# trevor-m/cuda-pathtrace

Measured on AMD Instinct MI355X. Metric: Msamples/s, 9-sphere Cornell box 1024x1024x1024spp, higher is better.
Workload: dtype f32+f64

## Files before the change

### cuda-pathtrace_amd/csrc/pt_grid.h

```cpp
#pragma once
#include "pt_intersect.h"

#pragma clang fp contract(off)

namespace pt {

#ifndef PT_V13_LAST_SHORTCUT
#define PT_V13_LAST_SHORTCUT 1
#endif
#ifndef PT_GRID_MAX_CELLS
#define PT_GRID_MAX_CELLS 4096
#endif
#ifndef PT_GRID_CELLS_PER_SPHERE
#define PT_GRID_CELLS_PER_SPHERE 2.75f
#endif
#ifndef PT_GRID_EXACT_REG
#define PT_GRID_EXACT_REG 1
#endif
constexpr int kGridMaxCells = PT_GRID_MAX_CELLS;
#ifndef PT_GRID_TESTS_PER_TRIP
#define PT_GRID_TESTS_PER_TRIP 3
#endif
#ifndef PT_GRID_MAX_ITEMS
#define PT_GRID_MAX_ITEMS 8192
// ... 469 lines not shown
    h.far2 = far * far;
    h.n_big = n_big | ((ncells + n_ext) << 16);
    h.n_items = total;
    h.r_small = r_small;
    h.r_big = r_big;
    h.prim_base = (uint32_t)max_entries;
    h.n_emis = s_n_emis > (uint32_t)kGridMaxEmis ? 0xFFFFu : s_n_emis;
    *hdr = h;
  }
}

#ifdef PT_GRID_STATS
__device__ unsigned long long g_grid_stats[8];
__device__ unsigned long long g_grid_hist[4][64];
#define PT_HIST_DECL int hist_tests = 0, hist_steps = 0, hist_trips = 0, hist_rounds = 0
#define PT_HIST_LANE(var, n) do { var += (n); } while (0)
#define PT_HIST_END(in_walk) do { \
    if (in_walk) { atomicAdd(&g_grid_hist[0][hist_tests < 63 ? hist_tests : 63], 1ull); atomicAdd(&g_grid_hist[1][hist_steps < 63 ? hist_steps : 63], 1ull); } \
    if ((threadIdx.x & 63) == __builtin_ctzll(__builtin_amdgcn_ballot_w64(true))) { \
      atomicAdd(&g_grid_hist[2][hist_trips < 63 ? hist_trips : 63], 1ull); atomicAdd(&g_grid_hist[3][hist_rounds < 63 ? hist_rounds : 63], 1ull); } } while (0)
#define PT_STAT(i, v) do { const unsigned long long v_ = (unsigned long long)(v);  \
    if ((threadIdx.x & 63) == __builtin_ctzll(__builtin_amdgcn_ballot_w64(true))) atomicAdd(&g_grid_stats[i], v_); } while (0)
#else
#define PT_STAT(i, v) do { } while (0)
#define PT_HIST_DECL
#define PT_HIST_LANE(var, n) do { } while (0)
#define PT_HIST_END(in_walk) do { } while (0)
#endif
#ifdef PT_GRID_STATS_AMBIG
#define PT_STATW(i, v) do { } while (0)
#else
#define PT_STATW(i, v) PT_STAT(i, v)
#endif
struct Near2 {
  float T1, T2;
  int i1;
};

template <bool ONCE = false>
__device__ __forceinline__ bool near2_test(Near2& s, const float4 g, int i, F3 o, F3 d, float a4, float Tlim_hi) {
  const float INF = __builtin_inff();
  const F3 off = mk3(o.x - g.x, o.y - g.y, o.z - g.z);
  const float b = 2.0f * dot(d, off);
  const float c = dot(off, off) - g.w;
  const float bb = b * b;
  const float a4c = a4 * c;
  const float dacc = fmaf(-a4, c, bb);
  const bool cand = ((int)__float_as_uint(dacc) >= 0) & (ONCE || !((i == s.i1) & (s.T1 < INF)));
  const float sq = __builtin_amdgcn_sqrtf(dacc);
  const float e = fmaf(b, b, -bb);
  const float num = a4c + e;
  const float TA = copysign_neg_b3(sq, b) - b;
  const float TB = num * __builtin_amdgcn_rcpf(TA);
  const uint32_t ta = __float_as_uint(TA), tb = __float_as_uint(TB);
  const uint32_t tbits = ta < tb ? ta : tb;
  const float T = __uint_as_float(tbits);
  const bool sure = fabsf(a4c) > fmaf(bb, 1.1920929e-07f, 1e-30f);
  const bool ok = cand & sure & (tbits < __float_as_uint(Tlim_hi));
  const float Te = ok ? T : INF;
  s.i1 = Te < s.T1 ? i : s.i1;
  s.T2 = __builtin_amdgcn_fmed3f(s.T1, s.T2, Te);
  s.T1 = fminf(s.T1, Te);
  return cand & !sure;
}

__device__ __forceinline__ void near2_exact(Near2& s, const float4 g, int i, F3 o, F3 d, float a, float Tlim_hi) {
// ... 105 lines not shown
    const float tn = par[k] ? (inside ? -INF : INF) : fminf(l, h);
    const float tf = par[k] ? (inside ? INF : -INF) : fmaxf(l, h);
    t_in = fmaxf(t_in, tn);
    t_out = fminf(t_out, tf);
  }
  active = (t_in <= t_out + slack_t) & (t_in * two_a < Tlim_hi);
  const int stride[3] = {1, dims[0], dims[0] * dims[1]};
#pragma unroll
  for (int k = 0; k < 3; k++) {
    const float p = oo[k] + dd[k] * t_in;
    int ci = (int)floorf((p - gmin[k]) * G.h.inv_cs);
    ci = ci < 0 ? 0 : (ci >= dims[k] ? dims[k] - 1 : ci);
    const bool fwd = dd[k] > 0.0f;
    const float bnd = gmin[k] + (float)(ci + (fwd ? 1 : 0)) * G.h.cs;
    const float tm = par[k] ? INF : (bnd - oo[k]) * inv[k];
    const float td = par[k] ? INF : G.h.cs * fabsf(inv[k]);
    if (k == 0) { w.tmax0 = tm; w.tdel0 = td; }
    if (k == 1) { w.tmax1 = tm; w.tdel1 = td; }
    if (k == 2) { w.tmax2 = tm; w.tdel2 = td; }
    cidx += ci * stride[k];
    const int sk = fwd ? stride[k] : -stride[k];
    if (k == 0) w.cs0 = sk;
    if (k == 1) w.cs1 = sk;
    if (k == 2) w.cs2 = sk;
    left |= (uint32_t)(fwd ? dims[k] - 1 - ci : ci) << (10 * k);
  }
  cidx = active ? cidx : 0;
  }
  w.cidx = cidx;
  w.left = left;
  w.e0 = 0u, w.e1 = 0u;
  w.k0 = 0u, w.k1 = 0u;
  if constexpr (POOLED) {
    const uint2 e = G.cells[prim ? G.h.prim_base + (uint32_t)kPrimEntriesPerLane * threadIdx.x : (uint32_t)cidx];
    active = active & !settled;
    w.e0 = (active | prim) ? e.x : 0u;
    w.e1 = e.y;
    active = active & !prim;
  } else {
    w.k0 = G.cell_start[cidx], w.k1 = G.cell_start[cidx + 1];
    if (!active) w.k1 = w.k0;
  }
  w.n0 = 0, w.n1 = 0;
  w.have_next = false;
#ifdef PT_TIMING_ONLY_NO_WALK
  active = false;
  w.k1 = w.k0;
  w.e0 = 0u;
#endif
  w.walking = active;
  w.t_box = t_out + 2.0f * slack_t;
  w.forced = false;
  PT_STAT(0, 1);
  PT_STAT(5, __builtin_popcountll(__builtin_amdgcn_ballot_w64(active)));
}

template <bool PARK>
__device__ __forceinline__ void grid_trips(GridWalk& walk, const GridLds& G, F3 o, F3 d, bool in_walk, bool alive, int park) {
  const float two_a = 2.0f * walk.a, a4 = 4.0f * walk.a;
  const float Tlim_hi = 1000000.0f * two_a * 1.0000153f;
  const float slack_t = G.h.slack * __builtin_amdgcn_rsqf(walk.a);
  Near2 s = walk.s;
  float tmax0 = walk.tmax0, tmax1 = walk.tmax1, tmax2 = walk.tmax2;
  const float tdel0 = walk.tdel0, tdel1 = walk.tdel1, tdel2 = walk.tdel2;
  int cidx = walk.cidx;
  const int cs0 = walk.cs0, cs1 = walk.cs1, cs2 = walk.cs2;
  uint32_t left = walk.left, k0 = walk.k0, k1 = walk.k1, n0 = walk.n0, n1 = walk.n1;
// ... 123 lines not shown
  const float INF = __builtin_inff();
  return (dot(oc, oc) <= G.h.far2) & (a > 0.0f) & (a < 1e30f) & (fabsf(d.x) < INF) & (fabsf(d.y) < INF) & (fabsf(d.z) < INF);
}

__device__ __forceinline__ bool intersect_scene_v11(const SceneLds& sc, int n, F3 o, F3 d, float& t_hit, int& idx) {
  if (n <= 0) return false;
  const float a = dot(d, d);
  const GridLds& G = *sc.grid;
  if (G.valid) {
    const bool admitted = grid_admits(G, o, d, a);
    PT_STATW(7, __builtin_amdgcn_ballot_w64(!admitted) != 0 ? 1 : 0);
    if (admitted) return intersect_scene_grid(sc, G, n, o, d, a, t_hit, idx);
  }
  return intersect_scene_screened_large(sc, n, o, d, make_ray_const(d), t_hit, idx);
}

#ifndef PT_POOL_STEPS
#define PT_POOL_STEPS 2
#endif
#ifdef PT_DEBUG_PIXEL
#define PT_DBG_ME() (blockIdx.x == PT_DEBUG_BLOCK && threadIdx.x == PT_DEBUG_THREAD)
#define PT_DBG_MY_WAVE() (blockIdx.x == PT_DEBUG_BLOCK && (threadIdx.x >> 6) == (PT_DEBUG_THREAD >> 6))
#define PT_DBG_OWNED(owner) (PT_DBG_MY_WAVE() && (owner) == (PT_DEBUG_THREAD & 63))
#define PT_DBG(...) do { printf(__VA_ARGS__); } while (0)
#else
#define PT_DBG_ME() false
#define PT_DBG_MY_WAVE() false
#define PT_DBG_OWNED(owner) false
#define PT_DBG(...) do { } while (0)
#endif
#ifndef PT_POOL_SCAN_DPP
#define PT_POOL_SCAN_DPP 1
#endif
#ifndef PT_POOL_SWEEP_BELOW
#define PT_POOL_SWEEP_BELOW 24
#endif
static_assert(63 + 64 * 3 * PT_POOL_STEPS + 2 <= kPoolRing, "pool ring too small");
static_assert(PT_POOL_STEPS == 1 || PT_POOL_STEPS == 2, "the link queue has two slots");

struct PoolLds {
  uint32_t* ring;
  unsigned long long* key1;
  uint32_t* t2;
  uint32_t* olist;
  unsigned long long* smask;
};
constexpr unsigned long long kPoolEmpty = 0x7F800000FFFFFFFFull;

__device__ __forceinline__ PoolLds pool_of_wave(void* workgroup_base) {
  char* b = reinterpret_cast<char*>(workgroup_base) + (threadIdx.x >> 6) * kPoolWaveBytes;
  PoolLds p;
  p.key1 = reinterpret_cast<unsigned long long*>(b);
  p.ring = reinterpret_cast<uint32_t*>(b + 64 * 8);
  p.t2 = reinterpret_cast<uint32_t*>(b + 64 * 8 + kPoolRing * 4);
  p.olist = p.t2 + 64;
  p.smask = reinterpret_cast<unsigned long long*>(p.olist + 64);
  return p;
}

__device__ __forceinline__ float bperm_f(int byte_addr, float v) {
  return __int_as_float(__builtin_amdgcn_ds_bpermute(byte_addr, __float_as_int(v)));
}

__device__ __forceinline__ bool dda_step(float& tmax0, float& tmax1, float& tmax2, float tdel0, float tdel1, float tdel2, int& cidx,
                                         int cs0, int cs1, int cs2, float tstop) {
  const float t_exit = fminf(fminf(tmax0, tmax1), tmax2);
  const bool a0 = (tmax0 <= tmax1) & (tmax0 <= tmax2);
  const bool a1 = !a0 & (tmax1 <= tmax2);
  tmax0 = a0 ? tmax0 + tdel0 : tmax0;
  tmax1 = a1 ? tmax1 + tdel1 : tmax1;
  tmax2 = (a0 | a1) ? tmax2 : tmax2 + tdel2;
  cidx += a0 ? cs0 : (a1 ? cs1 : cs2);
  return t_exit <= tstop;
}

__device__ __forceinline__ void grid_trips_pooled(GridWalk& walk, const GridLds& G, const PoolLds& P, F3 o, F3 d) {
  constexpr int K = PT_POOL_STEPS;
  const float INF = __builtin_inff();
  const int lane = threadIdx.x & 63;
  const float a4 = 4.0f * walk.a;
  const float two_a = 2.0f * walk.a;
  const float slack_t = G.h.slack * __builtin_amdgcn_rsqf(walk.a);
  const float Tcap = 1000000.0f * two_a * 1.0000153f;
  const float inv_two_a = __builtin_amdgcn_rcpf(two_a);
  float tmax0 = walk.tmax0, tmax1 = walk.tmax1, tmax2 = walk.tmax2;
  const float tdel0 = walk.tdel0, tdel1 = walk.tdel1, tdel2 = walk.tdel2;
  int cidx = walk.cidx;
  const int cs0 = walk.cs0, cs1 = walk.cs1, cs2 = walk.cs2;
  const uint32_t last_cell = G.h.nx * G.h.ny * G.h.nz - 1u;
  const float t_box = walk.t_box;
  auto stop_at = [&](float best) { return fminf(fmaf(fminf(best * 1.0000077f, Tcap), inv_two_a, slack_t), t_box) * 1.0000019f; };
  bool walking = walk.walking;
  int rounds_left = (int)(G.h.nx + G.h.ny + G.h.nz) / K + 8 + (int)((G.h.n_big >> 16) - (last_cell + 1u));
  const uint64_t here = __builtin_amdgcn_ballot_w64(true);
  const uint32_t rank = __builtin_amdgcn_mbcnt_hi((uint32_t)(here >> 32), __builtin_amdgcn_mbcnt_lo((uint32_t)here, 0u));
  const uint32_t n_here = (uint32_t)__builtin_popcountll(here);
  __hip_atomic_store(P.key1 + lane, walk.s.T1 < INF ? (((unsigned long long)__float_as_uint(walk.s.T1) << 32) | (uint32_t)walk.s.i1) : kPoolEmpty,
                     __ATOMIC_RELAXED, __HIP_MEMORY_SCOPE_WORKGROUP);
  __hip_atomic_store(P.t2 + lane, __float_as_uint(walk.s.T2), __ATOMIC_RELAXED, __HIP_MEMORY_SCOPE_WORKGROUP);
  uint32_t links = 0u;
  uint32_t tail = 0u;
  float tstop = stop_at(walk.s.T1);
  PT_HIST_DECL;
  if (PT_DBG_ME()) PT_DBG("ENTRY walking %d tmax %g %g %g tdel %g %g %g cidx %d cs %d %d %d tstop %g t_box %g e0 %08x e1 %08x n_here %u T1 %g o %g %g %g d %g %g %g\n", (int)walking, tmax0, tmax1, tmax2, tdel0, tdel1, tdel2, cidx, cs0, cs1, cs2, tstop, t_box, walk.e0, walk.e1, n_here, walk.s.T1, o.x, o.y, o.z, d.x, d.y, d.z);
  auto push = [&](uint32_t e0k, uint32_t e1k, uint32_t tag, bool first) {
    const uint64_t m1 = __builtin_amdgcn_ballot_w64(e0k >= 0x40000000u);
    if (m1 != 0) {
      const uint64_t m2 = __builtin_amdgcn_ballot_w64(e0k >= 0x80000000u), m3 = __builtin_amdgcn_ballot_w64(e0k >= 0xC0000000u);
      uint32_t pos = __builtin_amdgcn_mbcnt_hi((uint32_t)(m1 >> 32), __builtin_amdgcn_mbcnt_lo((uint32_t)m1, tail));
      pos = __builtin_amdgcn_mbcnt_hi((uint32_t)(m2 >> 32), __builtin_amdgcn_mbcnt_lo((uint32_t)m2, pos));
      pos = __builtin_amdgcn_mbcnt_hi((uint32_t)(m3 >> 32), __builtin_amdgcn_mbcnt_lo((uint32_t)m3, pos));
      PT_HIST_LANE(hist_tests, (int)(e0k >> 30));
      if (e0k >= 0x40000000u) {
        uint32_t* slot = P.ring + pos;
        slot[2] = tag | (e1k >> 16);
        asm volatile("" ::: "memory");
        slot[1] = tag | (e1k & 0xFFFFu);
        asm volatile("" ::: "memory");
        slot[0] = tag | (e0k & 0xFFFFu);
      }
      tail += (uint32_t)(__builtin_popcountll(m1) + __builtin_popcountll(m2) + __builtin_popcountll(m3));
      if (first) links |= e0k & 0x1FFF0000u; else links |= (e0k >> 16) & 0x1FFFu;
    }
  };
  auto drain = [&](bool fin) {
  if (tail >= (fin ? 1u : n_here)) {
    uint32_t head = 0u;
    do {
      const uint32_t n = (tail - head) < n_here ? (tail - head) : n_here;
      const bool valid = rank < n;
      PT_STATW(1, 1);
      PT_STATW(2, n);
      PT_HIST_LANE(hist_trips, 1);
      const uint32_t e = P.ring[head + rank];
      head += n;
      const int owner = valid ? (int)(e >> 16) : lane;
      const int i = valid ? (int)(e & 0xFFFFu) : 0;
      const float4 g = G.geom[i];
      const int oa = owner << 2;
      const F3 ro = mk3(bperm_f(oa, o.x), bperm_f(oa, o.y), bperm_f(oa, o.z));
      const F3 rd = mk3(bperm_f(oa, d.x), bperm_f(oa, d.y), bperm_f(oa, d.z));
      const float ra4 = bperm_f(oa, a4);
      const float rTlim_hi = 1000000.0f * (0.5f * ra4) * 1.0000153f;
      const F3 off = mk3(ro.x - g.x, ro.y - g.y, ro.z - g.z);
      const float b = 2.0f * dot(rd, off);
      const float cc = dot(off, off) - g.w;
      const float bb = b * b;
      const float a4c = ra4 * cc;
      const float dacc = fmaf(-ra4, cc, bb);
      const bool cand = valid & ((int)__float_as_uint(dacc) >= 0);
      const float sq = __builtin_amdgcn_sqrtf(dacc);
      const float ee = fmaf(b, b, -bb);
      const float num = a4c + ee;
      const float TA = copysign_neg_b3(sq, b) - b;
      const float TB = num * __builtin_amdgcn_rcpf(TA);
      const uint32_t ta = __float_as_uint(TA), tb = __float_as_uint(TB);
      const uint32_t tbits = ta < tb ? ta : tb;
      float T = __uint_as_float(tbits);
      const bool sure = fabsf(a4c) > fmaf(bb, 1.1920929e-07f, 1e-30f);
      bool ok = cand & sure & (tbits < __float_as_uint(rTlim_hi));
      if (__builtin_expect(cand & !sure, 0)) {
        float t = 0.0f;
        const float ra = 0.25f * ra4;
        const bool h = intersect_sphere(ro, rd, ra, g, t);
        T = (2.0f * ra) * t;
        ok = h & (t > 0.0f) & (T < rTlim_hi);
      }
      if (ok) {
        const unsigned long long key = ((unsigned long long)__float_as_uint(T) << 32) | (uint32_t)i;
        const unsigned long long old = __hip_atomic_fetch_min(P.key1 + owner, key, __ATOMIC_RELAXED, __HIP_MEMORY_SCOPE_WORKGROUP);
        if (old != key) {
          const unsigned long long loser = old > key ? old : key;
          __hip_atomic_fetch_min(P.t2 + owner, (uint32_t)(loser >> 32), __ATOMIC_RELAXED, __HIP_MEMORY_SCOPE_WORKGROUP);
        }
      }
    } while ((tail - head) >= (fin ? 1u : n_here));
    const uint32_t rest = tail - head;
    if (rest != 0u) {
      const uint32_t v = P.ring[head + (rank < rest ? rank : 0u)];
      if (rank < rest) P.ring[rank] = v;
    }
    tail = rest;
    tstop = stop_at(__uint_as_float(__hip_atomic_load(reinterpret_cast<uint32_t*>(P.key1 + lane) + 1, __ATOMIC_RELAXED, __HIP_MEMORY_SCOPE_WORKGROUP)));
  }
  };

  uint32_t e0[K], e1[K];
  e0[0] = walk.e0, e1[0] = walk.e1;
#pragma unroll
  for (int k = 1; k < K; k++) e0[k] = 0u, e1[k] = 0u;
  const uint32_t self = (uint32_t)lane << 16;
  bool sweep = false;
  for (;;) {
#pragma unroll
    for (int k = 0; k < K; k++) push(e0[k], e1[k], self, k == 0);
    const bool fin = __builtin_amdgcn_ballot_w64(walking | (links != 0u)) == 0;
    drain(fin);
    if (fin) break;
    if (__builtin_expect(--rounds_left < 0, 0)) {
      walk.forced = walk.forced | walking | (links != 0u);
      walking = false;
      links = 0u;
    }
    if (n_here == 64u && __builtin_amdgcn_ballot_w64(links != 0u) == 0 &&
        __builtin_popcountll(__builtin_amdgcn_ballot_w64(walking)) <= PT_POOL_SWEEP_BELOW) {
      if (PT_DBG_ME()) PT_DBG("SWITCH walking %d walkers %d tmax %g %g %g cidx %d tstop %g rounds_left %d\n", (int)walking, (int)__builtin_popcountll(__builtin_amdgcn_ballot_w64(walking)), tmax0, tmax1, tmax2, cidx, tstop, rounds_left);
      sweep = true;
      break;
    }
    PT_STATW(3, 1);
    PT_STATW(4, __builtin_popcountll(__builtin_amdgcn_ballot_w64(walking | (links != 0u))));
    PT_HIST_LANE(hist_rounds, 1);
    uint32_t cur = 0u;
    if (__builtin_amdgcn_ballot_w64(links != 0u) != 0) {
      const uint32_t hi = links >> 16;
      cur = hi != 0u ? hi : links;
      links = hi != 0u ? (links & 0xFFFFu) : 0u;
    }
#pragma unroll
    for (int k = 0; k < K; k++) e0[k] = 0u, e1[k] = 0u;
    const bool chain = cur != 0u;
    bool go = chain;
    if (!chain & walking) {
      PT_HIST_LANE(hist_steps, 1);
      walking = dda_step(tmax0, tmax1, tmax2, tdel0, tdel1, tdel2, cidx, cs0, cs1, cs2, tstop);
      go = walking;
    }
    if (go) {
      const uint32_t at = (uint32_t)cidx < last_cell ? (uint32_t)cidx : last_cell;
      const uint2 e = G.cells[chain ? cur : at];
      e0[0] = e.x, e1[0] = e.y;
    }
    if (PT_DBG_ME()) PT_DBG("STEP0 walking %d chain %d cidx %d entry %08x %08x tmax %g %g %g\n", (int)walking, (int)chain, cidx, e0[0], e1[0], tmax0, tmax1, tmax2);
#pragma unroll
    for (int k = 1; k < K; k++) {
      if (!chain & walking) {
        PT_HIST_LANE(hist_steps, 1);
        walking = dda_step(tmax0, tmax1, tmax2, tdel0, tdel1, tdel2, cidx, cs0, cs1, cs2, tstop);
        if (walking) {
          const uint32_t at = (uint32_t)cidx < last_cell ? (uint32_t)cidx : last_cell;
          const uint2 e = G.cells[at];
          e0[k] = e.x, e1[k] = e.y;
        }
      }
    }
    if (PT_DBG_ME()) PT_DBG("STEP1 walking %d cidx %d entry %08x %08x tmax %g %g %g\n", (int)walking, cidx, e0[K - 1], e1[K - 1], tmax0, tmax1, tmax2);
  }
  if (sweep) {
    uint32_t sw_n = 0u, sw_total = 0u, sw_done = 0u;
    bool wide = false;
    if (walking) {
      auto crossings = [&](float tm, float td) {
        const int n = tm <= tstop ? (int)((tstop - tm) * __builtin_amdgcn_rcpf(td)) + 1 : 0;
        return (uint32_t)(n < 0 ? 0 : n);
      };
      const uint32_t n0 = crossings(tmax0, tdel0), n1 = crossings(tmax1, tdel1), n2 = crossings(tmax2, tdel2);
      wide = (n0 | n1 | n2) > 255u;
      sw_n = n0 | (n1 << 8) | (n2 << 16) | (cs0 < 0 ? 1u << 24 : 0u) | (cs1 < 0 ? 1u << 25 : 0u) | (cs2 < 0 ? 1u << 26 : 0u);
      sw_total = n0 + n1 + n2;
      if (PT_DBG_ME()) PT_DBG("COUNTS n %u %u %u\n", n0, n1, n2);
    }
    if (__builtin_expect(__builtin_amdgcn_ballot_w64(wide) != 0, 0)) {
      walk.forced = walk.forced | walking;
      sw_total = 0u;
    }
    uint32_t se0 = 0u, se1 = 0u, tag = self;
    for (;;) {
      se0 = 0u, se1 = 0u;
      if (__builtin_amdgcn_ballot_w64(links != 0u) != 0) {
        if (links != 0u) {
          const uint32_t hi = links >> 16, cur = hi != 0u ? hi : links;
          links = hi != 0u ? (links & 0xFFFFu) : 0u;
          const uint2 e = G.cells[cur];
          se0 = e.x, se1 = e.y;
        }
      } else {
        const uint32_t rem = sw_total - sw_done;
        uint32_t incl = rem;
#if PT_POOL_SCAN_DPP
// ... 31 lines not shown
        const bool serving = (uint32_t)lane < (served < 64u ? served : 64u);
        PT_STATW(3, 1);
        PT_STATW(4, served < 64u ? served : 64u);
        sw_done += take;
        const uint32_t info = P.olist[serving ? ray : 0u];
        const int oa = (int)(info & 0xFFu) << 2;
        const float m0 = bperm_f(oa, tmax0), m1 = bperm_f(oa, tmax1), m2 = bperm_f(oa, tmax2);
        const float d0 = bperm_f(oa, tdel0), d1 = bperm_f(oa, tdel1), d2 = bperm_f(oa, tdel2);
        const int base = __builtin_amdgcn_ds_bpermute(oa, cidx);
        const uint32_t nn = (uint32_t)__builtin_amdgcn_ds_bpermute(oa, (int)sw_n);
        if (serving) {
          const uint32_t li = (info >> 16) + ((uint32_t)lane - ((info >> 8) & 0xFFu));
          const uint32_t n0 = nn & 0xFFu, n1 = (nn >> 8) & 0xFFu;
          const bool k0 = li < n0, k1 = !k0 & (li < n0 + n1);
          const uint32_t i = li - (k0 ? 0u : (k1 ? n0 : n0 + n1));
          const float tc = (k0 ? m0 : (k1 ? m1 : m2)) + (float)i * (k0 ? d0 : (k1 ? d1 : d2));
          const int ax = k0 ? 0 : (k1 ? 1 : 2);
          auto taken = [&](float tmx, float td, int m) {
            const int j = tc >= tmx ? (int)((tc - tmx) * __builtin_amdgcn_rcpf(td) + 0.75f) : 0;
            const float tj = tmx + (float)j * td;
            return ((tj < tc) | ((tj == tc) & (m < ax))) ? j + 1 : j;
          };
          const int c0 = k0 ? (int)i + 1 : taken(m0, d0, 0), c1 = k1 ? (int)i + 1 : taken(m1, d1, 1),
                    c2 = (k0 | k1) ? taken(m2, d2, 2) : (int)i + 1;
          const int sx = (int)G.h.nx, sxy = (int)(G.h.nx * G.h.ny);
          const int idx = base + ((nn >> 24) & 1u ? -c0 : c0) + ((nn >> 25) & 1u ? -c1 : c1) * sx + ((nn >> 26) & 1u ? -c2 : c2) * sxy;
          const uint32_t at = (uint32_t)idx < last_cell ? (uint32_t)idx : last_cell;
          const uint2 e = G.cells[at];
          se0 = e.x, se1 = e.y;
          tag = (info & 0xFFu) << 16;
          if (PT_DBG_OWNED(info & 0xFFu)) PT_DBG("SERVE helper %d li %u axis %d i %u tc %g c %d %d %d base %d idx %d entry %08x %08x nn %08x\n", lane, li, k0 ? 0 : (k1 ? 1 : 2), i, tc, c0, c1, c2, base, idx, e.x, e.y, nn);
        }
      }
      push(se0, se1, tag, true);
      const bool fin = __builtin_amdgcn_ballot_w64((links != 0u) | (sw_done < sw_total)) == 0;
      drain(fin);
      if (fin) break;
    }
  }
  PT_HIST_END(true);
  const unsigned long long k = __hip_atomic_load(P.key1 + lane, __ATOMIC_RELAXED, __HIP_MEMORY_SCOPE_WORKGROUP);
  walk.s.T1 = __uint_as_float((uint32_t)(k >> 32));
  walk.s.i1 = walk.s.T1 < INF ? (int)(uint32_t)k : 0;
  walk.s.T2 = __uint_as_float(__hip_atomic_load(P.t2 + lane, __ATOMIC_RELAXED, __HIP_MEMORY_SCOPE_WORKGROUP));
  if (PT_DBG_ME()) PT_DBG("FINAL T1 %g i1 %d T2 %g forced %d swept %d\n", walk.s.T1, walk.s.i1, walk.s.T2, (int)walk.forced, (int)sweep);
}

__device__ __forceinline__ bool intersect_scene_grid_pooled(const SceneLds& sc, const GridLds& G, int n, F3 o, F3 d, float a,
                                                            float& t_hit, int& idx, bool walker = true, bool prim = false,
                                                            bool last = false) {
  GridWalk w;
  grid_begin<true>(w, G, o, d, a, prim & walker, last & walker);
  const float INF = __builtin_inff();
  w.s.T1 = walker ? w.s.T1 : INF;
  w.s.T2 = walker ? w.s.T2 : INF;
  w.walking = w.walking & walker;
  w.e0 = walker ? w.e0 : 0u;
  w.e1 = walker ? w.e1 : 0u;
  grid_trips_pooled(w, G, pool_of_wave(sc.pool), o, d);
  if (!walker) return false;
  return grid_end(w, sc, G, n, o, d, t_hit, idx);
}

__device__ __forceinline__ bool intersect_scene_v13(const SceneLds& sc, int n, F3 o, F3 d, float& t_hit, int& idx, bool live = true,
                                                    bool prim = false, bool last = false) {
  if (n <= 0) return false;
  const float a = dot(d, d);
  const GridLds& G = *sc.grid;
  if (G.valid) {
    const bool admitted = live && grid_admits(G, o, d, a);
    PT_STATW(7, __builtin_amdgcn_ballot_w64(live & !admitted) != 0 ? 1 : 0);
    const bool walk_here = __builtin_amdgcn_ballot_w64(admitted) != 0;
    if (admitted | (walk_here & !live)) {
// ... 10 lines not shown
```

### cuda-pathtrace_amd/csrc/pt_kernel.hip

```cpp
#include "pt_trace.h"

#pragma clang fp contract(off)

static constexpr int kNumVariants = 15;
static constexpr int kT = PT_BLOCK_THREADS, kTG = PT_GRID_BLOCK_THREADS, kTW = PT_GRID_WIDE_THREADS;
static constexpr int kW = PT_MIN_WAVES, kWG = PT_GRID_MIN_WAVES, kWD = PT_GRID12_MIN_WAVES, kWP = PT_POOL_MIN_WAVES;
static constexpr VariantInfo kVariants[kNumVariants] = {
     {true,  1, kT,  PT_LEAN_NEVER,  PT_LDS_PLAIN,  PT_GRID_NONE,   false, false, false, false, PT_CHUNK_NONE,     false, kW,   PT_LOOP_SAMPLES,   0,     0},
     {false, 1, kT,  PT_LEAN_NEVER,  PT_LDS_PLAIN,  PT_GRID_NONE,   false, false, false, false, PT_CHUNK_NONE,     false, kW,   PT_LOOP_SAMPLES,   1,     1},
     {false, 1, kT,  PT_LEAN_NEVER,  PT_LDS_PLAIN,  PT_GRID_NONE,   false, false, false, false, PT_CHUNK_NONE,     false, kW,   PT_LOOP_SAMPLES,   2,     2},
     {false, 1, kT,  PT_LEAN_NEVER,  PT_LDS_PACKED, PT_GRID_NONE,   false, false, false, false, PT_CHUNK_NONE,     false, kW,   PT_LOOP_SAMPLES,   3,     3},
     {false, 1, kT,  PT_LEAN_NEVER,  PT_LDS_PLAIN,  PT_GRID_NONE,   false, false, false, false, PT_CHUNK_NONE,     false, kW,   PT_LOOP_SAMPLES,   4,     4},
     {false, 1, kT,  PT_LEAN_NEVER,  PT_LDS_PLAIN,  PT_GRID_NONE,   false, false, false, false, PT_CHUNK_NONE,     false, kW,   PT_LOOP_SAMPLES,   5,     5},
     {true,  1, kT,  PT_LEAN_BIG,    PT_LDS_WALLS,  PT_GRID_NONE,   false, true,  true,  true,  PT_CHUNK_ONE_LANE, true,  kW,   PT_LOOP_SAMPLES,   6,     6},
     {false, 1, kT,  PT_LEAN_NEVER,  PT_LDS_PLAIN,  PT_GRID_NONE,   false, false, false, false, PT_CHUNK_NONE,     false, kW,   PT_LOOP_PAIRS,     6,     7},
     {true,  4, kT,  PT_LEAN_BIG,    PT_LDS_PLAIN,  PT_GRID_NONE,   false, true,  false, false, PT_CHUNK_SPLIT,    true,  0,    PT_LOOP_SAMPLES,   6,     8},
     {true,  2, kT,  PT_LEAN_NEVER,  PT_LDS_PLAIN,  PT_GRID_NONE,   false, true,  false, false, PT_CHUNK_SPLIT,    true,  0,    PT_LOOP_SAMPLES,   6,     9},
     {true,  1, kT,  PT_LEAN_BIG,    PT_LDS_PLAIN,  PT_GRID_NONE,   false, false, true,  false, PT_CHUNK_NONE,     false, kW,   PT_LOOP_REGEN,     6,     10},
     {false, 1, kTG, PT_LEAN_ALWAYS, PT_LDS_PLAIN,  PT_GRID_LANE,   false, false, false, false, PT_CHUNK_NONE,     false, kWG,  PT_LOOP_REGEN,     11,    11},
     {false, 1, kTG, PT_LEAN_ALWAYS, PT_LDS_PLAIN,  PT_GRID_LANE,   false, false, false, false, PT_CHUNK_NONE,     false, kWD,  PT_LOOP_DECOUPLED, 11,    12},
     {true,  1, kTG, PT_LEAN_ALWAYS, PT_LDS_PLAIN,  PT_GRID_POOLED, false, false, true,  false, PT_CHUNK_GRID,     true,  kWP,  PT_LOOP_REGEN,     13,    13},
     {true,  1, kTW, PT_LEAN_ALWAYS, PT_LDS_PLAIN,  PT_GRID_POOLED, true,  false, true,  false, PT_CHUNK_GRID,     false, kWP,  PT_LOOP_REGEN,     13,    13},
};
static constexpr VariantInfo kNoVariant = {false, 1, kT, PT_LEAN_NEVER, PT_LDS_PLAIN, PT_GRID_NONE, false, false, false, false, PT_CHUNK_NONE, false, kW, PT_LOOP_SAMPLES, 0, 0};
// ... 249 lines not shown
      sx /= (float)a.height;
      sy /= (float)a.width;
    }
    dir = lerp(lerp(B0, B1, sy), lerp(B2, B3, sy), 1.0f - sx);
  };

  auto dir_at = [&](float sx, float sy) {
    if (pow2_image) {
      sx *= inv_h;
      sy *= inv_w;
    } else {
      sx /= (float)a.height;
      sy /= (float)a.width;
    }
    return lerp(lerp(B0, B1, sy), lerp(B2, B3, sy), 1.0f - sx);
  };
  if constexpr (REF) {
#ifndef PT_NO_FOOTPRINT
    if (pass_spp >= PT_FOOTPRINT_MIN_SPP) {
      const uint32_t mine = active ? primary_candidates(sc, a.n_spheres, (float)row, (float)col, dir_at) : 0u;
      uint32_t wave_mask = 0u;
#pragma unroll
      for (int j = 0; j < 9; j++) wave_mask |= (__builtin_amdgcn_ballot_w64(((mine >> j) & 1u) != 0u) != 0ull) ? (1u << j) : 0u;
      sc.prim_mask = wave_mask;
    }
#endif
  }

  int i = active ? i_begin : i_end;
  bool prim_ok = false;
  if constexpr (POOLED && PT_PRIMLIST) {
    if (grid.valid && pass_spp >= PT_PRIMLIST_MIN_SPP && a.max_bounces >= 1) {
      int k = 0;
      const uint32_t slot = grid.h.prim_base + (uint32_t)kPrimEntriesPerLane * threadIdx.x;
      prim_ok = build_primary_list(grid, a.spheres, a.n_spheres, eye, (float)row, (float)col, active, dir_at, pool_of_wave(sc.pool).ring,
                                   const_cast<uint2*>(grid.cells), slot, k);
      if (prim_ok & (k == 0) & ((grid.h.n_big & 0xFFFFu) == 0u)) {
        for (; i < i_end; i++) {
          if constexpr (RNG == PT_RNG_XORWOW) {
            if (RESUME || a.spp != 1) {
              float jx, jy;
              rng.jitter(jx, jy);
            }
          }
          L.color = L.color + mk3(0.0f, 0.0f, 0.0f);
        }
      }
    }
  }
  if constexpr (kRegen) {
    int n = 0;
    F3 o = eye, d = eye;
    F3 color = mk3(0.0f, 0.0f, 0.0f), mask = mk3(1.0f, 1.0f, 1.0f);
    const int span = i_end - i_begin;
    const bool by_progress = span >= PT_PRIO_MIN_SPP_REGEN;
    const int q1 = i_begin + span / 4, q2 = i_begin + span / 2, q3 = i_end - span / 4;
    int last_band = -1;
    for (;;) {
      const bool live = i < i_end;
      if constexpr (POOLED && PT_POOL_HELPERS) {
        if (__builtin_amdgcn_ballot_w64(live) == 0) break;
      } else {
        if (!live) break;
      }
      if (by_progress) {
        int iu;
        if constexpr (POOLED && PT_POOL_HELPERS) iu = __builtin_amdgcn_readlane(i, __builtin_ctzll(__builtin_amdgcn_ballot_w64(live)));
        else iu = __builtin_amdgcn_readfirstlane(i);
        const int band = (iu >= q1 ? 1 : 0) + (iu >= q2 ? 1 : 0) + (iu >= q3 ? 1 : 0);
// ... 655 lines not shown
  return (const void*)select_kernel<>(rng_mode, run_variant(variant, max_bounces), n_spheres, max_bounces, planar);
}
const void* pt_resume_kernel_symbol(int rng_mode, int variant, int n_spheres, int max_bounces, bool planar) {
  return (const void*)select_kernel<false, true>(rng_mode, variant, n_spheres, max_bounces, planar);
}
const void* pt_adaptive_kernel_symbol(int rng_mode, int variant, int n_spheres, int max_bounces, bool planar) {
  return (const void*)select_kernel<false, true, true>(rng_mode, variant, n_spheres, max_bounces, planar);
}

#ifdef PT_SCREEN_STATS
extern "C" int pt_debug_screen_stats(unsigned long long out[8], int reset) {
  unsigned long long zero[8] = {0, 0, 0, 0, 0, 0, 0, 0};
  if (hipMemcpyFromSymbol(out, HIP_SYMBOL(pt::g_screen_stats), sizeof(zero)) != hipSuccess) return -2;
  if (reset && hipMemcpyToSymbol(HIP_SYMBOL(pt::g_screen_stats), zero, sizeof(zero)) != hipSuccess) return -2;
  return 0;
}
#endif

#ifdef PT_GRID_STATS
extern "C" int pt_debug_grid_hist(unsigned long long out[256], int reset) {
  static unsigned long long zero[256];
  if (hipMemcpyFromSymbol(out, HIP_SYMBOL(pt::g_grid_hist), sizeof(zero)) != hipSuccess) return -2;
  if (reset && hipMemcpyToSymbol(HIP_SYMBOL(pt::g_grid_hist), zero, sizeof(zero)) != hipSuccess) return -2;
  return 0;
}
extern "C" int pt_debug_grid_stats(unsigned long long out[8], int reset) {
  unsigned long long zero[8] = {0, 0, 0, 0, 0, 0, 0, 0};
  if (hipMemcpyFromSymbol(out, HIP_SYMBOL(pt::g_grid_stats), sizeof(zero)) != hipSuccess) return -2;
  if (reset && hipMemcpyToSymbol(HIP_SYMBOL(pt::g_grid_stats), zero, sizeof(zero)) != hipSuccess) return -2;
  return 0;
}
#endif

size_t pt_kernel_accel_bytes(void) { return pt::kGridAccelBytes; }

int pt_kernel_max_spheres(int variant) {
  const VariantInfo& v = pt_kernel_variant(variant);
  if (v.lean != PT_LEAN_NEVER) return 1 << 26;
  const size_t fixed = tail_lds_bytes(0, v) + pt::kTablesF4 * sizeof(float4);
  if (v.lds_extra == PT_LDS_PACKED) return (int)((PT_LDS_BUDGET_BYTES - fixed - 2 * sizeof(float4)) / (5 * sizeof(float4)));
  return (int)((PT_LDS_BUDGET_BYTES - fixed) / (4 * sizeof(float4)));
}

hipError_t pt_launch_build_grid(const pt_sphere* spheres, int n, uint32_t* accel, const float* eye, bool pooled, hipStream_t stream, int threads) {
  hipLaunchKernelGGL(pt::build_grid_kernel, dim3(1), dim3(pt::kGridBuildThreads), 0, stream, spheres, n, accel, eye ? eye[0] : 0.0f,
                     eye ? eye[1] : 0.0f, eye ? eye[2] : 0.0f, eye ? 1 : 0, pt::grid_max_entries(n, pooled, threads));
  return hipGetLastError();
}

void pt_kernel_grid_layout(int n_spheres, int threads, uint64_t out[8]) {
  out[0] = pt::kGridAccelBytes;
  out[1] = pt::kGridBigOff;
  out[2] = pt::kGridStartOff;
  out[3] = pt::kGridItemsOff;
  out[4] = pt::kGridCellsOff;
  out[5] = pt::kGridEmisOff;
  out[6] = (uint64_t)pt::kGridMaxCells;
  out[7] = (uint64_t)pt::grid_max_entries(n_spheres, true, threads);
}

bool pt_kernel_chunked(int variant, int n_spheres, int max_bounces, bool planar, int spp, uint32_t chunks) {
  const VariantInfo& v = pt_kernel_variant(variant);
  const bool build_chunks = v.chunk_build(!lds_lean(n_spheres, v) && ref_config(n_spheres, max_bounces, v, planar));
  return build_chunks && chunks > 1u && chunks <= (uint32_t)PT_CHUNKS_MAX && spp >= 2 * (int)chunks &&
         (spp + (int)chunks - 1) / (int)chunks <= (v.chunk_family == PT_CHUNK_GRID ? PT_CHUNK_MAX_SAMPLES_GRID : PT_CHUNK_MAX_SAMPLES);
}
// ... 220 lines not shown
```

### cuda-pathtrace_amd/csrc/pt_primlist.h

```cpp
#pragma once
#include "pt_grid.h"
#include "pt_footprint.h"

#pragma clang fp contract(off)

namespace pt {

#ifndef PT_PRIMLIST
#define PT_PRIMLIST 1
#endif
#ifndef PT_PRIMLIST_MIN_SPP
#define PT_PRIMLIST_MIN_SPP 4
#endif
constexpr int kPrimMaxSurvivors = 256;
static_assert(kPrimMaxSurvivors <= kPoolRing, "the survivor list lives in the test ring");

#if defined(PT_PRIMLIST_MUTANT) && PT_PRIMLIST_MUTANT == 1
constexpr float kPrimRadiusFactor = 0.3f;
constexpr double kPrimMissScale = 1.0;
#elif defined(PT_PRIMLIST_MUTANT) && PT_PRIMLIST_MUTANT == 2
constexpr float kPrimRadiusFactor = 1.05f;
constexpr double kPrimMissScale = 0.64;
#else
constexpr float kPrimRadiusFactor = 1.05f;
constexpr double kPrimMissScale = 1.0;
#endif

__device__ __forceinline__ bool prim_cone_excludes(const float4 g, F3 eye, F3 axis, float rho) {
  const F3 off = mk3(eye.x - g.x, eye.y - g.y, eye.z - g.z);
  const double ox = off.x, oy = off.y, oz = off.z, ux = axis.x, uy = axis.y, uz = axis.z;
  const double o2 = ox * ox + oy * oy + oz * oz, uu = ux * ux + uy * uy + uz * uz, hu = ux * ox + uy * oy + uz * oz;
  const double rr = (double)g.w * kPrimMissScale;
  const double lo = sqrt(o2), lu = sqrt(uu);
  const double p2 = o2 - hu * hu / uu;
  const double q = sqrt(p2 > 0.0 ? p2 : 0.0) - (double)rho * lo;
  const bool miss = (q > 0.0) & (q * q - rr > 4.76837158203125e-06 * o2);
  const bool behind = (o2 - rr >= 0.00390625 * o2) & (hu > (double)rho * lo * lu * 1.000001);
  return miss | behind;
}

template <typename DirFn>
__device__ __forceinline__ bool build_primary_list(const GridLds& G, const pt_sphere* __restrict__ spheres, int n, F3 eye,
                                                   float row, float col, bool active, DirFn dir_at, uint32_t* ring, uint2* cells,
                                                   uint32_t slot, int& k_out) {
  const int lane = threadIdx.x & 63;
  k_out = 0;
  const F3 dc = dir_at(row, col);
  const float lc = sqrtf(dot(dc, dc));
  float dev = 0.0f;
#pragma unroll
  for (int k = 0; k < 4; k++) {
    const F3 dk = dir_at(row + ((k & 1) ? 0.5f : -0.5f), col + ((k & 2) ? 0.5f : -0.5f));
    const F3 e = dk - dc;
    const float len = sqrtf(dot(e, e));
    dev = !(len <= dev) ? len : dev;
  }
  const float rho = kPrimRadiusFactor * dev / lc + 1e-6f;
  bool ok = active & (rho <= 0.125f) & (lc > 0.0f) & (dev >= 0.0f);
  const F3 u = dc * (1.0f / lc);
  const uint64_t okm = __builtin_amdgcn_ballot_w64(ok);
  uint32_t n_surv = 0u;
  bool wave_ok = okm != 0ull;
  if (wave_ok) {
    const int l0 = __builtin_ctzll(okm), l1 = 63 - __builtin_clzll(okm);
    auto rl = [](float v, int l) { return __int_as_float(__builtin_amdgcn_readlane(__float_as_int(v), l)); };
    F3 A = mk3(rl(u.x, l0) + rl(u.x, l1), rl(u.y, l0) + rl(u.y, l1), rl(u.z, l0) + rl(u.z, l1));
    A = A * (1.0f / sqrtf(dot(A, A)));
    const F3 e = u - A;
    float wr = ok ? 1.05f * sqrtf(dot(e, e)) + rho : 0.0f;
#pragma unroll
    for (int m = 1; m < 64; m <<= 1) wr = fmaxf(wr, __shfl_xor(wr, m));
    wave_ok = (wr <= 0.25f) & (wr > 0.0f);
    if (wave_ok) {
      for (int j0 = 0; j0 < n; j0 += 64) {
        const int j = j0 + lane;
        bool keep = false;
        if (j < n) {
// ... 5 lines not shown
        const uint32_t pos = n_surv + __builtin_amdgcn_mbcnt_hi((uint32_t)(km >> 32), __builtin_amdgcn_mbcnt_lo((uint32_t)km, 0u));
        if (keep && pos < (uint32_t)kPrimMaxSurvivors) ring[pos] = (uint32_t)j;
        n_surv += (uint32_t)__builtin_popcountll(km);
      }
      wave_ok = n_surv <= (uint32_t)kPrimMaxSurvivors;
    }
  }
  ok = ok & wave_ok;
  unsigned long long lo64 = 0ull;
  uint32_t hi16 = 0u;
  int k = 0;
  if (wave_ok) {
    asm volatile("" ::: "memory");
    for (uint32_t s = 0; s < n_surv; s++) {
      const uint32_t j = ring[s];
      const bool keep = ok && !prim_cone_excludes(G.geom[j], eye, dc, rho);
      if (keep) {
        hi16 = (uint32_t)(lo64 >> 48);
        lo64 = (lo64 << 16) | j;
        k++;
      }
    }
    asm volatile("" ::: "memory");
  }
  ok = ok & (k <= kPrimMaxList);
  const uint32_t kk = ok ? (uint32_t)k : 0u;
  const uint32_t s0 = (uint32_t)lo64 & 0xFFFFu, s1 = (uint32_t)(lo64 >> 16) & 0xFFFFu, s2 = (uint32_t)(lo64 >> 32) & 0xFFFFu,
                 s3 = (uint32_t)(lo64 >> 48), s4 = hi16 & 0xFFFFu;
  uint2 e0, e1;
  if (kk <= 3u) {
    e0 = make_uint2(s0 | (kk << 30), s1 | (s2 << 16));
    e1 = make_uint2(0u, 0u);
  } else {
    e0 = make_uint2(s0 | ((slot + 1u) << 16) | (2u << 30), s1);
    e1 = make_uint2(s2 | ((kk - 2u) << 30), s3 | (s4 << 16));
  }
  cells[slot] = e0;
  cells[slot + 1u] = e1;
  k_out = (int)kk;
  return ok;
}

}
```

Measured before the change: 24730.

## Prefetch next pool ring entry, recompute ray a4, stride primary-list LDS slots

The pooled drain loop now reads the next ring entry one pass ahead so the LDS load latency overlaps the intersection arithmetic, and the compaction reuses the prefetched value. The per-owner a4 is recomputed from the gathered direction instead of being fetched with an extra bpermute. Primary-list cell entries are laid out with a block-wide stride instead of adjacent pairs, which is meant to reduce LDS bank conflicts. Optional timestamp instrumentation is added behind a macro. The read-ahead can touch up to 63 slots past the ring's last entry, which a new static assert guards.

```diff
diff --git a/cuda-pathtrace_amd/csrc/pt_grid.h b/cuda-pathtrace_amd/csrc/pt_grid.h
--- a/cuda-pathtrace_amd/csrc/pt_grid.h
+++ b/cuda-pathtrace_amd/csrc/pt_grid.h
@@ -525,6 +525,33 @@
 #else
 #define PT_STATW(i, v) PT_STAT(i, v)
 #endif
+#ifdef PT_WALK_STAMPS
+enum { kStampPush, kStampGather, kStampArith, kStampAtomics, kStampCompact, kStampSteps, kStampSweep, kStampWalk, kStampPieces };
+constexpr int kStampRows = 1024;
+__device__ unsigned long long g_walk_stamps[kStampRows][kStampPieces][2];
+struct WalkClock {
+  unsigned long long t0, last;
+  uint32_t cyc[kStampPieces], cnt[kStampPieces];
+};
+__device__ __forceinline__ unsigned long long walk_now() {
+  __builtin_amdgcn_sched_barrier(0);
+  asm volatile("s_waitcnt lgkmcnt(0)" ::: "memory");
+  const unsigned long long t = __builtin_amdgcn_s_memtime();
+  __builtin_amdgcn_sched_barrier(0);
+  return t;
+}
+#define PT_CLOCK_BEGIN WalkClock wc; do { for (int k_ = 0; k_ < kStampPieces; k_++) wc.cyc[k_] = 0u, wc.cnt[k_] = 0u; wc.t0 = wc.last = walk_now(); } while (0)
+#define PT_CLOCK(k) do { const unsigned long long t_ = walk_now(); wc.cyc[k] += (uint32_t)(t_ - wc.last); wc.cnt[k] += 1u; wc.last = t_; } while (0)
+#define PT_CLOCK_END do { wc.cyc[kStampWalk] = (uint32_t)(walk_now() - wc.t0); wc.cnt[kStampWalk] = 1u; \
+    if ((threadIdx.x & 63) == __builtin_ctzll(__builtin_amdgcn_ballot_w64(true))) { \
+      const uint32_t row_ = (blockIdx.x * (blockDim.x >> 6) + (threadIdx.x >> 6)) & (uint32_t)(kStampRows - 1); \
+      _Pragma("unroll") for (int k_ = 0; k_ < kStampPieces; k_++) { \
+        atomicAdd(&g_walk_stamps[row_][k_][0], (unsigned long long)wc.cyc[k_]); atomicAdd(&g_walk_stamps[row_][k_][1], (unsigned long long)wc.cnt[k_]); } } } while (0)
+#else
+#define PT_CLOCK_BEGIN do { } while (0)
+#define PT_CLOCK(k) do { } while (0)
+#define PT_CLOCK_END do { } while (0)
+#endif
 struct Near2 {
   float T1, T2;
   int i1;
@@ -696,7 +723,7 @@
   w.e0 = 0u, w.e1 = 0u;
   w.k0 = 0u, w.k1 = 0u;
   if constexpr (POOLED) {
-    const uint2 e = G.cells[prim ? G.h.prim_base + (uint32_t)kPrimEntriesPerLane * threadIdx.x : (uint32_t)cidx];
+    const uint2 e = G.cells[prim ? G.h.prim_base + threadIdx.x : (uint32_t)cidx];
     active = active & !settled;
     w.e0 = (active | prim) ? e.x : 0u;
     w.e1 = e.y;
@@ -886,10 +913,14 @@
 #ifndef PT_POOL_SCAN_DPP
 #define PT_POOL_SCAN_DPP 1
 #endif
+#ifndef PT_POOL_READ_AHEAD
+#define PT_POOL_READ_AHEAD 1
+#endif
 #ifndef PT_POOL_SWEEP_BELOW
 #define PT_POOL_SWEEP_BELOW 24
 #endif
 static_assert(63 + 64 * 3 * PT_POOL_STEPS + 2 <= kPoolRing, "pool ring too small");
+static_assert(63 + 64 * 3 * PT_POOL_STEPS + 63 < kPoolRing, "the drain reads one pass ahead: up to 63 slots past the ring's last entry");
 static_assert(PT_POOL_STEPS == 1 || PT_POOL_STEPS == 2, "the link queue has two slots");
 
 struct PoolLds {
@@ -932,7 +963,6 @@
   constexpr int K = PT_POOL_STEPS;
   const float INF = __builtin_inff();
   const int lane = threadIdx.x & 63;
-  const float a4 = 4.0f * walk.a;
   const float two_a = 2.0f * walk.a;
   const float slack_t = G.h.slack * __builtin_amdgcn_rsqf(walk.a);
   const float Tcap = 1000000.0f * two_a * 1.0000153f;
@@ -956,6 +986,7 @@
   uint32_t tail = 0u;
   float tstop = stop_at(walk.s.T1);
   PT_HIST_DECL;
+  PT_CLOCK_BEGIN;
   if (PT_DBG_ME()) PT_DBG("ENTRY walking %d tmax %g %g %g tdel %g %g %g cidx %d cs %d %d %d tstop %g t_box %g e0 %08x e1 %08x n_here %u T1 %g o %g %g %g d %g %g %g\n", (int)walking, tmax0, tmax1, tmax2, tdel0, tdel1, tdel2, cidx, cs0, cs1, cs2, tstop, t_box, walk.e0, walk.e1, n_here, walk.s.T1, o.x, o.y, o.z, d.x, d.y, d.z);
   auto push = [&](uint32_t e0k, uint32_t e1k, uint32_t tag, bool first) {
     const uint64_t m1 = __builtin_amdgcn_ballot_w64(e0k >= 0x40000000u);
@@ -980,13 +1011,18 @@
   auto drain = [&](bool fin) {
   if (tail >= (fin ? 1u : n_here)) {
     uint32_t head = 0u;
+#if PT_POOL_READ_AHEAD
+    uint32_t e = P.ring[rank];
+#endif
     do {
       const uint32_t n = (tail - head) < n_here ? (tail - head) : n_here;
       const bool valid = rank < n;
       PT_STATW(1, 1);
       PT_STATW(2, n);
       PT_HIST_LANE(hist_trips, 1);
+#if !PT_POOL_READ_AHEAD
       const uint32_t e = P.ring[head + rank];
+#endif
       head += n;
       const int owner = valid ? (int)(e >> 16) : lane;
       const int i = valid ? (int)(e & 0xFFFFu) : 0;
@@ -994,7 +1030,13 @@
       const int oa = owner << 2;
       const F3 ro = mk3(bperm_f(oa, o.x), bperm_f(oa, o.y), bperm_f(oa, o.z));
       const F3 rd = mk3(bperm_f(oa, d.x), bperm_f(oa, d.y), bperm_f(oa, d.z));
-      const float ra4 = bperm_f(oa, a4);
+#if PT_POOL_READ_AHEAD
+      e = P.ring[head + rank];
+      const float ra4 = 4.0f * dot(rd, rd);
+#else
+      const float ra4 = bperm_f(oa, 4.0f * walk.a);
+#endif
+      PT_CLOCK(kStampGather);
       const float rTlim_hi = 1000000.0f * (0.5f * ra4) * 1.0000153f;
       const F3 off = mk3(ro.x - g.x, ro.y - g.y, ro.z - g.z);
       const float b = 2.0f * dot(rd, off);
@@ -1020,6 +1062,7 @@
         T = (2.0f * ra) * t;
         ok = h & (t > 0.0f) & (T < rTlim_hi);
       }
+      PT_CLOCK(kStampArith);
       if (ok) {
         const unsigned long long key = ((unsigned long long)__float_as_uint(T) << 32) | (uint32_t)i;
         const unsigned long long old = __hip_atomic_fetch_min(P.key1 + owner, key, __ATOMIC_RELAXED, __HIP_MEMORY_SCOPE_WORKGROUP);
@@ -1028,14 +1071,20 @@
           __hip_atomic_fetch_min(P.t2 + owner, (uint32_t)(loser >> 32), __ATOMIC_RELAXED, __HIP_MEMORY_SCOPE_WORKGROUP);
         }
       }
+      PT_CLOCK(kStampAtomics);
     } while ((tail - head) >= (fin ? 1u : n_here));
     const uint32_t rest = tail - head;
+#if PT_POOL_READ_AHEAD
+    if (rank < rest) P.ring[rank] = e;
+#else
     if (rest != 0u) {
       const uint32_t v = P.ring[head + (rank < rest ? rank : 0u)];
       if (rank < rest) P.ring[rank] = v;
     }
+#endif
     tail = rest;
     tstop = stop_at(__uint_as_float(__hip_atomic_load(reinterpret_cast<uint32_t*>(P.key1 + lane) + 1, __ATOMIC_RELAXED, __HIP_MEMORY_SCOPE_WORKGROUP)));
+    PT_CLOCK(kStampCompact);
   }
   };
 
@@ -1048,6 +1097,7 @@
   for (;;) {
 #pragma unroll
     for (int k = 0; k < K; k++) push(e0[k], e1[k], self, k == 0);
+    PT_CLOCK(kStampPush);
     const bool fin = __builtin_amdgcn_ballot_w64(walking | (links != 0u)) == 0;
     drain(fin);
     if (fin) break;
@@ -1099,6 +1149,7 @@
       }
     }
     if (PT_DBG_ME()) PT_DBG("STEP1 walking %d cidx %d entry %08x %08x tmax %g %g %g\n", (int)walking, cidx, e0[K - 1], e1[K - 1], tmax0, tmax1, tmax2);
+    PT_CLOCK(kStampSteps);
   }
   if (sweep) {
     uint32_t sw_n = 0u, sw_total = 0u, sw_done = 0u;
@@ -1196,13 +1247,16 @@
           if (PT_DBG_OWNED(info & 0xFFu)) PT_DBG("SERVE helper %d li %u axis %d i %u tc %g c %d %d %d base %d idx %d entry %08x %08x nn %08x\n", lane, li, k0 ? 0 : (k1 ? 1 : 2), i, tc, c0, c1, c2, base, idx, e.x, e.y, nn);
         }
       }
+      PT_CLOCK(kStampSweep);
       push(se0, se1, tag, true);
+      PT_CLOCK(kStampPush);
       const bool fin = __builtin_amdgcn_ballot_w64((links != 0u) | (sw_done < sw_total)) == 0;
       drain(fin);
       if (fin) break;
     }
   }
   PT_HIST_END(true);
+  PT_CLOCK_END;
   const unsigned long long k = __hip_atomic_load(P.key1 + lane, __ATOMIC_RELAXED, __HIP_MEMORY_SCOPE_WORKGROUP);
   walk.s.T1 = __uint_as_float((uint32_t)(k >> 32));
   walk.s.i1 = walk.s.T1 < INF ? (int)(uint32_t)k : 0;
diff --git a/cuda-pathtrace_amd/csrc/pt_kernel.hip b/cuda-pathtrace_amd/csrc/pt_kernel.hip
--- a/cuda-pathtrace_amd/csrc/pt_kernel.hip
+++ b/cuda-pathtrace_amd/csrc/pt_kernel.hip
@@ -305,9 +305,9 @@
   if constexpr (POOLED && PT_PRIMLIST) {
     if (grid.valid && pass_spp >= PT_PRIMLIST_MIN_SPP && a.max_bounces >= 1) {
       int k = 0;
-      const uint32_t slot = grid.h.prim_base + (uint32_t)kPrimEntriesPerLane * threadIdx.x;
+      const uint32_t slot = grid.h.prim_base + threadIdx.x;
       prim_ok = build_primary_list(grid, a.spheres, a.n_spheres, eye, (float)row, (float)col, active, dir_at, pool_of_wave(sc.pool).ring,
-                                   const_cast<uint2*>(grid.cells), slot, k);
+                                   const_cast<uint2*>(grid.cells), slot, (uint32_t)blockDim.x, k);
       if (prim_ok & (k == 0) & ((grid.h.n_big & 0xFFFFu) == 0u)) {
         for (; i < i_end; i++) {
           if constexpr (RNG == PT_RNG_XORWOW) {
@@ -1029,6 +1029,20 @@
 }
 #endif
 
+#ifdef PT_WALK_STAMPS
+extern "C" int pt_debug_walk_stamps(unsigned long long out[16], int reset) {
+  static_assert(pt::kStampPieces == 8, "tools/walk_stamps.py names eight pieces");
+  static unsigned long long rows[pt::kStampRows][16], zero[pt::kStampRows][16];
+  if (hipMemcpyFromSymbol(rows, HIP_SYMBOL(pt::g_walk_stamps), sizeof(rows)) != hipSuccess) return -2;
+  if (reset && hipMemcpyToSymbol(HIP_SYMBOL(pt::g_walk_stamps), zero, sizeof(zero)) != hipSuccess) return -2;
+  for (int k = 0; k < 16; k++) {
+    out[k] = 0;
+    for (int r = 0; r < pt::kStampRows; r++) out[k] += rows[r][k];
+  }
+  return 0;
+}
+#endif
+
 size_t pt_kernel_accel_bytes(void) { return pt::kGridAccelBytes; }
 
 int pt_kernel_max_spheres(int variant) {
diff --git a/cuda-pathtrace_amd/csrc/pt_primlist.h b/cuda-pathtrace_amd/csrc/pt_primlist.h
--- a/cuda-pathtrace_amd/csrc/pt_primlist.h
+++ b/cuda-pathtrace_amd/csrc/pt_primlist.h
@@ -42,7 +42,7 @@
 template <typename DirFn>
 __device__ __forceinline__ bool build_primary_list(const GridLds& G, const pt_sphere* __restrict__ spheres, int n, F3 eye,
                                                    float row, float col, bool active, DirFn dir_at, uint32_t* ring, uint2* cells,
-                                                   uint32_t slot, int& k_out) {
+                                                   uint32_t slot, uint32_t stride, int& k_out) {
   const int lane = threadIdx.x & 63;
   k_out = 0;
   const F3 dc = dir_at(row, col);
@@ -114,11 +114,11 @@
     e0 = make_uint2(s0 | (kk << 30), s1 | (s2 << 16));
     e1 = make_uint2(0u, 0u);
   } else {
-    e0 = make_uint2(s0 | ((slot + 1u) << 16) | (2u << 30), s1);
+    e0 = make_uint2(s0 | ((slot + stride) << 16) | (2u << 30), s1);
     e1 = make_uint2(s2 | ((kk - 2u) << 30), s3 | (s4 << 16));
   }
   cells[slot] = e0;
-  cells[slot + 1u] = e1;
+  cells[slot + stride] = e1;
   k_out = (int)kk;
   return ok;
 }
```

New measurement: 24640. No clear change (-0.3%).
